# parseablehq/parseable

Hardware: AMD Instinct MI355X
Metric: rows/sec scanned (SELECT...WHERE...GROUP BY, Parseable parquet dialect) (higher is better)
Workload: dtype int64; 1 GPU; c2s; query=SELECT host,count(*),max(latency) WHERE ts BETWEEN ... GROUP BY host, rows_per_gpu=100000000, parallelism=dp1

## Files before the change

parseable_amd/csrc/gpuq.cpp:

```cpp
#include "../../include/gpuq.h"
#include "catalog.h"
#include "where.h"
#include "meta.h"
#include "kernels_api.h"
#include "dev_types.h"
#include "like.h"

#include <hip/hip_runtime.h>
#include <fcntl.h>
#include <sys/mman.h>
#include <sys/stat.h>
#include <unistd.h>

#include <algorithm>
#include <array>
#include <atomic>
#include <functional>
#include <cstring>
#include <thread>
#include <map>
#include <memory>
#include <mutex>
#include <string>
#include <unordered_map>
// ... 175 lines not shown
struct RgRef {
  int file_idx, rg_idx;
  int64_t rows = 0, needed_bytes = 0, total_bytes = 0;
  uint32_t row_start = 0;
};

enum TaskKind { TK_DICT_GID, TK_DICT_VAL, TK_PLAIN_VAL, TK_DELTA_VAL,
                TK_DICT_MASK, TK_BYTES_CONTAINS, TK_POOL_VAL,
                TK_IS_NULL, TK_IS_NOT_NULL,
                TK_N };
constexpr int TK_CTX_SHIFT = 8;
inline int tk_ctx(int kind, int ctx) { return kind | (ctx << TK_CTX_SHIFT); }
inline int tk_kind(int key) { return key & ((1 << TK_CTX_SHIFT) - 1); }
inline int tk_ctx_of(int key) { return key >> TK_CTX_SHIFT; }

struct Partition {
  int device = -1;
  std::vector<RgRef> rgs;
  int64_t n_rows = 0;
  std::vector<ChunkTask> chunks;
  std::vector<DevPage> pages;
  std::map<std::pair<int,int>, std::vector<int32_t>> tasks;
  std::vector<int32_t> remap_pool;
  std::vector<int64_t> dictv_pool;
  std::vector<uint8_t> lut_pool;
  std::vector<std::vector<uint8_t>> lut_pool_x;
  std::vector<DevSeg> segs;
  std::vector<DevBr> brs;
  std::vector<DevPageBr> pagebrs;
  std::vector<DevBrRes> res_lane, res_wave;
  std::vector<DevPiece> piece_pool;
  std::vector<DevSeq> seqs;
  std::vector<DevSeqTile> tiles;
  std::vector<DevLit> lits_wave;
  std::vector<DevCWin> cwins;
  std::vector<uint16_t> cstarts;
  std::map<int, std::pair<uint32_t, uint32_t>> cwin_ranges;
  uint64_t raw_bytes = 0, dec_bytes = 0;
  int64_t bytes_scanned = 0, rowgroup_bytes_total = 0;
  int64_t bytes_cache_hit = 0;
  bool populated = false;
  std::map<int, std::vector<std::pair<int64_t, int64_t>>> pred_ranges;
  std::vector<std::pair<uint64_t, std::vector<uint8_t>>> himgs;

  bool loaded = false;
  hipStream_t stream = nullptr;
  uint8_t *d_raw = nullptr, *d_dec = nullptr;
  DevPage* d_pages = nullptr;
  int32_t* d_remap = nullptr;
  int64_t* d_dictv = nullptr;
  uint8_t* d_lut = nullptr;
  uint8_t* d_mask = nullptr;
  std::vector<uint8_t*> d_fbufs;
  std::vector<uint8_t*> d_wbufs;
  int32_t* d_err = nullptr;
  uint64_t* d_table = nullptr;
  uint64_t* d_fsum = nullptr;
  uint64_t* d_hkeys = nullptr;
  int32_t* d_hgids = nullptr;
  uint32_t* d_hcount = nullptr;
  std::map<int, uint64_t*> d_gid2ref;
// ... 78 lines not shown
  std::vector<Partition> parts;
  int32_t n_groups = 0;
  int32_t n_fsum = 0;
  bool has_hash = false;
  bool needs_cascade = false;
  bool has_numkey = false;
  std::vector<std::string> pinned_keys;
  int64_t m_cache_hit_bytes = 0;
  bool fused_count = false;
  bool fused_valagg = false;
  int valagg_col = -1;
  bool valagg_late = false;
  int valagg_blocks = 1024;
  bool no_fused_valagg = false;
  bool dict_serial = false;
  bool exec_dbg = false;
  std::vector<int> distinct_aggs;
  bool has_tree = false;
  WhereTree where;
  std::vector<int> pred_ctx;
  struct WOr { int node; int ctx; int level; std::vector<int> terms; };
  struct WFold { int node; int ctx; int col; };
  struct WCtx { std::vector<int> ors; };
  std::vector<WCtx> ctxs;
  std::vector<WOr> wors;
  std::vector<WFold> wfolds;
  int n_wbufs = 0;
  int ctx_of(int pidx) const { return has_tree ? pred_ctx[pidx] : 0; }
  bool no_fcount = false;
  struct AggFilter { int agg; int root; int ctx; int depth; };
// ... 22 lines not shown
extern "C" void gpuq_session_destroy(gpuq_ctx* c) { delete c; }
namespace {
thread_local std::string g_null_ctx_error = "null ctx";
}
extern "C" const char* gpuq_last_error(gpuq_ctx* c) {
  return c ? c->last_error.c_str() : g_null_ctx_error.c_str();
}
extern "C" int32_t gpuq_device_count(void) {
  int n = 0;
  if (hipGetDeviceCount(&n) != hipSuccess) return -1;
  return n;
}

namespace {

void read_env_knobs(gpuq_plan* plan) {
  plan->exec_dbg = getenv("GPUQ_PLAN_DEBUG") != nullptr;
  plan->no_fused_valagg = getenv("GPUQ_NO_FUSED_VALAGG") != nullptr;
  plan->no_fcount = getenv("GPUQ_NO_FCOUNT") != nullptr;
  if (const char* e = getenv("GPUQ_VALAGG_BLOCKS"))
    plan->valagg_blocks = std::max(1, atoi(e));
  if (const char* e = getenv("GPUQ_DICT_WALK"))
    plan->dict_serial = strcmp(e, "serial") == 0;
  if (const char* e = getenv("GPUQ_DISTINCT_BITMAP_BITS"))
    plan->distinct_bitmap_bits =
        std::min<uint64_t>(strtoull(e, nullptr, 10), 1ull << 31);
  if (const char* e = getenv("GPUQ_DISTINCT_LDS_BITS"))
    plan->distinct_lds_bits =
        std::min<uint64_t>(strtoull(e, nullptr, 10), 64 * 1024 * 8);
  if (const char* e = getenv("GPUQ_DISTINCT_PAIR_CAP"))
    plan->distinct_pair_cap = (uint32_t)std::min<uint64_t>(
        std::max<uint64_t>(strtoull(e, nullptr, 10), 1), DISTINCT_PAIR_CAP);
  if (const char* e = getenv("GPUQ_DISTINCT_FORCE_HASH"))
    plan->distinct_force_hash = atoi(e) != 0;
}

int find_or_add_col(std::vector<ColPlan>& cols, const std::string& name) {
  for (size_t i = 0; i < cols.size(); i++)
// ... 329 lines not shown
    const std::vector<T>& s = cbs[i].*src;
    for (size_t j = 0; j < s.size(); j++) {
      T e = s[j];
      rebase(e, i);
      dst[off[i] + j] = e;
    }
  });
  return off;
}
template <class C, class T, class B>
std::vector<size_t> merge_stream(std::vector<C>& cbs, std::vector<T> B::*src,
                                 std::vector<T>& dst) {
  return merge_stream(cbs, src, dst, [](T&, size_t) {});
}

Ring::Ring(hipStream_t st) : stream(st) {
  for (int i = 0; i < NBUF; i++) {
    HIP_TRY(hipHostMalloc(&bufs[i], BUFSZ));
    HIP_TRY(hipEventCreate(&evts[i]));
    HIP_TRY(hipEventRecord(evts[i], stream));
  }
}
Ring::~Ring() {
  for (int i = 0; i < NBUF; i++) {
    if (bufs[i]) (void)hipHostFree(bufs[i]);
    if (evts[i]) (void)hipEventDestroy(evts[i]);
  }
}
void Ring::copy_spans(uint8_t* d_dst, const std::vector<Span>& spans) {
  size_t si = 0;
// ... 17 lines not shown
      if (soff == spans[si].len) { si++; soff = 0; }
    }
    parallel_for(fills.size(), [&](size_t f) {
      memcpy(fills[f].dstp, fills[f].src, fills[f].len);
    }, 32);
    HIP_TRY(hipMemcpyAsync(d_dst + dst, bufs[b], filled,
                           hipMemcpyHostToDevice, stream));
    HIP_TRY(hipEventRecord(evts[b], stream));
    dst += filled;
    b = (b + 1) % NBUF;
  }
}
void Ring::copy(void* d_dst, const void* src, size_t len) {
  if (len) copy_spans((uint8_t*)d_dst, {{(const uint8_t*)src, len}});
}

struct DecompRecs {
  std::vector<DevSeg> segs;
  std::vector<DevBr> brs;
  std::vector<DevPageBr> pagebrs;
  std::vector<DevBrRes> res_lane, res_wave;
  std::vector<DevPiece> piece_pool;
  std::vector<DevSeq> seqs;
  std::vector<DevSeqTile> tiles;
  std::vector<DevLit> lits_wave;
  std::vector<std::pair<uint64_t, std::vector<uint8_t>>> himgs;
};

constexpr uint32_t BR_FAR = 16384 / 2;

void plan_decomp_page(DecompRecs& cb, int codec, const uint8_t* praw,
                      uint64_t src_abs, uint64_t dst_abs, uint32_t comp,
                      uint32_t uncomp, bool raw_page,
                      int force = GPUQ_DECOMP_AUTO,
                      gpuq_decomp_stats* st = nullptr) {
  Lz4Plan lp;
  if (st) *st = gpuq_decomp_stats{};
  if (!raw_page && codec == CODEC_SNAPPY) {
    lp = snappy_walk(praw, comp, uncomp);
    if (st) st->n_seq = lp.n_seq;
    if (lp.fallback) {
      std::vector<uint8_t> img(uncomp);
// ... 166 lines not shown
      }
      push_seq(dst_abs + lt.dst, rec, len);
    } else {
      const Lz4Resolved& rr = lp.resolved[ri++];
      if (try_inline(rr, &pat, &period)) {
        push_seq(dst_abs + rr.dst, {src_abs | match_bits(rr.len, period), pat},
                 rr.len);
        if (st) st->n_inl++;
      } else {
        push_resolved(rr);
      }
    }
  }
}

struct DecompDev {
  const uint8_t* d_raw;
  uint8_t* d_dec;
  const DevSeg* d_segs; int n_segs;
  const DevSeq* d_seqs;
  const DevSeqTile* d_tiles; int n_tiles;
  const DevLit* d_lits_wave; int n_lits_wave;
  const DevBrRes* d_res_lane; int64_t n_res_lane;
  const DevBrRes* d_res_wave; int n_res_wave;
  const DevPiece* d_piece_pool;
  const DevBr* d_brs;
  const DevPageBr* d_pagebrs; int n_pagebrs;
  int32_t* d_err;
};

void launch_decompress(hipStream_t st, const DecompDev& d) {
  launch_lz4_seg(st, d.d_raw, d.d_dec, d.d_segs, d.n_segs, d.d_err);
  launch_seq_tile(st, d.d_raw, d.d_dec, d.d_seqs, d.d_tiles, d.n_tiles);
  launch_lit_wave(st, d.d_raw, d.d_dec, d.d_lits_wave, d.n_lits_wave);
  launch_brres_lane(st, d.d_dec, d.d_res_lane, d.d_piece_pool, d.n_res_lane);
  launch_brres_wave(st, d.d_dec, d.d_res_wave, d.d_piece_pool, d.n_res_wave);
  launch_lz4_backrefs(st, d.d_dec, d.d_brs, d.d_pagebrs, d.n_pagebrs);
}

void plan_debug_report(gpuq_plan* plan,
                       std::map<size_t, std::array<int64_t, 3>>& null_dbg,
                       const std::vector<std::array<int64_t, 2>>& leaf_dbg,
                       const std::vector<char>& or_path) {
  fprintf(stderr, "[gpuq plan] fused_count=%d fused_valagg=%d%s\n",
          (int)plan->fused_count, (int)plan->fused_valagg,
          plan->fused_valagg && plan->valagg_late
              ? " (group count checked at execute)" : "");
  for (int ai : plan->distinct_aggs) {
// ... 7 lines not shown
    size_t period_le3 = 0;
    for (const DevSeq& r : pt.seqs) {
      const uint32_t ml = (uint32_t)(r.a >> 49) & 0x1ff;
      const uint32_t n = std::min(ml, (uint32_t)(r.a >> 58));
      for (uint32_t q = 1; q <= 3 && ml; q++) {
        bool ok = true;
        for (uint32_t j = q; j < n && ok; j++)
          ok = (uint8_t)(r.pat >> (j * 8)) == (uint8_t)(r.pat >> ((j - q) * 8));
        if (ok) { period_le3++; break; }
      }
    }
    fprintf(stderr,
            "[gpuq plan] part %zu: rows=%lld chunks=%zu pages=%zu segs=%zu "
            "tiles=%zu tile_recs=%zu period_le3=%zu lits_wave=%zu "
            "res=%zu/%zu pieces=%zu raw=%.2fGB "
            "dec=%.2fGB cwins=%zu\n",
            p, (long long)pt.n_rows, pt.chunks.size(), pt.pages.size(),
            pt.segs.size(), pt.tiles.size(), pt.seqs.size(), period_le3,
            pt.lits_wave.size(), pt.res_lane.size(), pt.res_wave.size(),
            pt.piece_pool.size(), pt.raw_bytes / 1e9, pt.dec_bytes / 1e9,
            pt.cwins.size());
  }
  for (size_t pi = 0; pi < plan->preds.size(); pi++) {
    const auto& pp = plan->preds[pi];
    std::string path;
    if (op_is_like(pp.p.op)) {
      int ci = find_or_add_col(plan->cols, pp.col);
      if (plan->cols[ci].hash_mode) {
        path = "hash";
      } else {
        bool lut = false, win = false;
        int k = plan->ctx_of((int)pi);
        if (k < 0)
          for (auto& f : plan->wfolds)
            if (f.col == ci) k = f.ctx;
        for (auto& part : plan->parts) {
// ... 914 lines not shown
          } else throw std::runtime_error("unsupported encoding for string predicate");
        }
        for (auto& nt : stubs[ti].null_tasks)
          cb.tasks[{tk_ctx(nt.first, nt.second), t.col_idx}].push_back(this_pid);
        cb.pages.push_back(dp);
      }
      if (row_in_rg != (uint32_t)mf.meta.row_groups[t.rg_idx].num_rows)
        throw std::runtime_error("page rows mismatch");
    });

    phase_mark("phase4 lz4 walks");

    {
      const size_t nc = cbs.size();
      merge_stream(cbs, &CB::pages, part.pages);
      merge_stream(cbs, &CB::segs, part.segs);
      const auto o_brs = merge_stream(cbs, &CB::brs, part.brs);
      merge_stream(cbs, &CB::pagebrs, part.pagebrs,
                   [&](DevPageBr& pb, size_t i) {
                     pb.start += (uint32_t)o_brs[i];
                   });
      const auto o_pp = merge_stream(cbs, &CB::piece_pool, part.piece_pool);
      auto piece_rebase = [&](DevBrRes& r, size_t i) {
        r.piece_start += (uint32_t)o_pp[i];
      };
      merge_stream(cbs, &CB::res_lane, part.res_lane, piece_rebase);
      merge_stream(cbs, &CB::res_wave, part.res_wave, piece_rebase);
      const auto o_sq = merge_stream(cbs, &CB::seqs, part.seqs);
      merge_stream(cbs, &CB::tiles, part.tiles,
                   [&](DevSeqTile& t, size_t i) { t.rec0 += o_sq[i]; });
      merge_stream(cbs, &CB::lits_wave, part.lits_wave);
      for (size_t i = 0; i < nc; i++) {
        auto& cb = cbs[i];
        for (auto& [key, ids] : cb.tasks) {
          auto& dstv = part.tasks[key];
          dstv.insert(dstv.end(), ids.begin(), ids.end());
        }
        citems.insert(citems.end(), cb.citems.begin(), cb.citems.end());
        for (auto& h : cb.himgs)
          part.himgs.emplace_back(h.first, std::move(h.second));
      }
    }
    phase_mark("phase5 merge");
    part.dec_bytes += 16384 + 64;

    if (!citems.empty()) {
// ... 276 lines not shown
  if (ctx) ctx->set_error(e.what());
  return nullptr;
}

extern "C" int32_t gpuq_plan_partition_count(gpuq_plan* p) {
  return p ? (int32_t)p->parts.size() : 0;
}

extern "C" int32_t gpuq_plan_load(gpuq_plan* plan, int32_t pi) try {
  if (!plan || pi < 0 || pi >= (int32_t)plan->parts.size()) return -1;
  Partition& part = plan->parts[pi];
  if (part.loaded) return 0;
  int64_t t0 = now_ns();
  HIP_TRY(hipSetDevice(part.device));
  HIP_TRY(hipStreamCreateWithFlags(&part.stream, hipStreamNonBlocking));

  HIP_TRY(hipMalloc(&part.d_raw, std::max<uint64_t>(part.raw_bytes + 8192, 16)));
  HIP_TRY(hipMalloc(&part.d_dec, std::max<uint64_t>(part.dec_bytes, 16)));
  Ring ring(part.stream);
  {
    std::vector<Ring::Span> run;
    uint64_t run_dst = 0, cursor = 0;
    auto flush = [&]() {
      if (!run.empty()) {
        ring.copy_spans(part.d_raw + run_dst, run);
        run.clear();
      }
    };
    for (auto& t : part.chunks) {
      const auto& mf = *plan->files[t.file_idx];
// ... 145 lines not shown
              (void**)&part.d_brs);
  upload_pool(part.pagebrs.data(), part.pagebrs.size() * sizeof(DevPageBr),
              (void**)&part.d_pagebrs);
  upload_pool(part.res_lane.data(), part.res_lane.size() * sizeof(DevBrRes),
              (void**)&part.d_res_lane);
  upload_pool(part.res_wave.data(), part.res_wave.size() * sizeof(DevBrRes),
              (void**)&part.d_res_wave);
  upload_pool(part.piece_pool.data(), part.piece_pool.size() * sizeof(DevPiece),
              (void**)&part.d_piece_pool);
  upload_pool(part.seqs.data(), part.seqs.size() * sizeof(DevSeq),
              (void**)&part.d_seqs);
  upload_pool(part.tiles.data(), part.tiles.size() * sizeof(DevSeqTile),
              (void**)&part.d_tiles);
  upload_pool(part.lits_wave.data(), part.lits_wave.size() * sizeof(DevLit),
              (void**)&part.d_lits_wave);
  upload_pool(part.cwins.data(), part.cwins.size() * sizeof(DevCWin),
              (void**)&part.d_cwins);
  upload_pool(part.cstarts.data(), part.cstarts.size() * sizeof(uint16_t),
              (void**)&part.d_cstarts);
  std::string needle;
  part.needle_off.assign(plan->preds.size(), 0);
  {
    std::string pool;
    for (size_t i = 0; i < plan->preds.size(); i++) {
      if (plan->preds[i].p.lit_kind == GPUQ_LIT_STR) {
        part.needle_off[i] = (uint32_t)pool.size();
        pool += plan->preds[i].str_lit;
        pool.push_back('\0');
      }
    }
// ... 352 lines not shown
      ch->buffers[1] = v;
    }
  }
  s->cursor += k;
  return 0;
} catch (const std::exception& e) {
  auto* s = (ProjState*)st0->private_data;
  s->err = e.what();
  return 1;
}

}

struct ExecEvents {
  hipEvent_t ev0 = nullptr, ev1 = nullptr, decomp = nullptr;
  ExecEvents() = default;
  ExecEvents(const ExecEvents&) = delete;
  ExecEvents& operator=(const ExecEvents&) = delete;
  void create() {
    HIP_TRY(hipEventCreate(&ev0));
    HIP_TRY(hipEventCreate(&ev1));
    HIP_TRY(hipEventCreate(&decomp));
  }
  ~ExecEvents() {
    for (hipEvent_t e : {ev0, ev1, decomp})
      if (e) (void)hipEventDestroy(e);
  }
};

int cmp_mode_of(int op) {
  switch (op) {
    case GPUQ_EQ: return CMP_EQ;
    case GPUQ_NE: return CMP_NE;
    case GPUQ_LT: return CMP_LT;
    case GPUQ_LE: return CMP_LE;
    case GPUQ_GT: return CMP_GT;
    case GPUQ_GE: return CMP_GE;
    default: return -1;
  }
}
// ... 192 lines not shown
  bool cascaded = false;
  std::vector<uint32_t> level_claimed;
  std::vector<char> distinct_bitmap(plan->distinct_aggs.size(), 0);
  auto key_card = [&](int ci) -> int64_t {
    const auto& kc = plan->cols[ci];
    return kc.is_bin ? (int64_t)kc.nbins + 1
           : (kc.hash_mode || kc.numeric_key)
               ? (int64_t)part.hash_claimed[ci] + 1
               : (int64_t)kc.gdict.size() + 1;
  };
  if (plan->fused_count)
    launch_init_table(st, part.d_table, plan->n_groups, (int)plan->aggs.size(),
                      part.d_agg_kind);

  HIP_TRY(hipEventRecord(ev0, st));
  launch_decompress(st, DecompDev{
      part.d_raw, part.d_dec,
      part.d_segs, (int)part.segs.size(),
      part.d_seqs, part.d_tiles, (int)part.tiles.size(),
      part.d_lits_wave, (int)part.lits_wave.size(),
      part.d_res_lane, (int64_t)part.res_lane.size(),
      part.d_res_wave, (int)part.res_wave.size(),
      part.d_piece_pool, part.d_brs,
      part.d_pagebrs, (int)part.pagebrs.size(), part.d_err});
  HIP_TRY(hipEventRecord(ev_decomp, st));

  if (plan->fused_count) {
    int key_col = plan->group_cols[0];
    auto it = part.tasks.find({TK_DICT_GID, key_col});
    if (it != part.tasks.end())
      launch_dict_count(st, part.d_dec, part.d_pages, part.d_ids[it->first],
                        (int)it->second.size(), part.d_remap, part.d_table,
                        plan->n_groups, (int)plan->aggs.size(), part.d_err);
    HIP_TRY(hipEventRecord(ev1, st));
  } else {
  auto run_task = [&](const std::pair<const std::pair<int, int>,
                                      std::vector<int32_t>>& kv,
                      uint8_t* mk) {
    const int kind = tk_kind(kv.first.first), kctx = tk_ctx_of(kv.first.first);
    const int col = kv.first.second;
    int n = (int)kv.second.size();
    int32_t* ids = part.d_ids[kv.first];
    const uint8_t* d_lut = part.d_lut;
    if (plan->exec_dbg &&
        (kind == TK_DICT_GID || kind == TK_DICT_VAL || kind == TK_DICT_MASK))
      fprintf(stderr,
              "[gpuq exec] part %d: dict decode col=%s pages=%d dict_walk=%s\n",
              pi, plan->cols[col].name.c_str(), n,
// ... 87 lines not shown
                          part.d_tmpvalid, mk, nullptr, nullptr,
                          part.d_present, part.d_err);
        break;
      case TK_IS_NULL:
        launch_def_levels(st, part.d_dec, part.d_pages, ids, n,
                          part.d_tmpvalid, nullptr, nullptr, nullptr,
                          part.d_present, part.d_err);
        launch_null_clear_valid(st, part.d_dec, part.d_pages, ids, n,
                                part.d_tmpvalid, mk);
        break;
    }
  };
  for (auto& kv : part.tasks) {
    if (plan->fused_valagg && kv.first.second == plan->valagg_col) continue;
    if (tk_ctx_of(kv.first.first) != 0) continue;
    run_task(kv, part.d_mask);
  }
  if (plan->has_hash || plan->has_numkey) {
    std::vector<int> gid_cols = plan->group_cols;
    for (int ai : plan->distinct_aggs) {
      int ci = plan->aggs[ai].col_idx;
      if (std::find(gid_cols.begin(), gid_cols.end(), ci) == gid_cols.end())
        gid_cols.push_back(ci);
    }
    for (int ci : gid_cols) {
      auto& c = plan->cols[ci];
      if (!c.hash_mode && !c.numeric_key) continue;
      reset_hash_table(part, st, (1ull << HASH_LOG2) + 1);
      auto itv = part.d_valid.find(ci);
      uint8_t* v = itv != part.d_valid.end() ? itv->second : nullptr;
// ... 23 lines not shown
      if (!c.hash_mode || c.lut_preds.empty()) continue;
      for (int pidx : c.lut_preds) {
        if (plan->ctx_of(pidx) != k) continue;
        const auto& pp = plan->preds[pidx];
        int op = cmp_mode_of(pp.p.op);
        if (op < 0) op = cmp_str_like(like_mode(pp.p.op));
        auto itv = part.d_valid.find((int)ci);
        launch_cmp_str(st, part.d_dec, part.d_val[(int)ci],
                       itv != part.d_valid.end() ? itv->second : nullptr,
                       part.d_needle + part.needle_off[pidx],
                       (uint32_t)pp.str_lit.size(), op, mk,
                       part.n_rows);
      }
    }

    for (size_t ci = 0; ci < plan->cols.size(); ci++) {
      auto& c = plan->cols[ci];
      for (int pidx : c.cmp_preds) {
        if (plan->ctx_of(pidx) != k) continue;
        const auto& pp = plan->preds[pidx];
        int mode = pp.p.op == GPUQ_BETWEEN ? CMP_RANGE : cmp_mode_of(pp.p.op);
        if (mode < 0) throw std::runtime_error("bad cmp op");
        int is_f64 = (c.phys == PT_DOUBLE) ? 1 : 0;
        int64_t lo = pp.p.i64[0], hi = pp.p.i64[1];
        if (is_f64) {
          memcpy(&lo, &pp.p.f64[0], 8);
          memcpy(&hi, &pp.p.f64[1], 8);
        }
        auto rit = part.pred_ranges.find(pidx);
        if (rit == part.pred_ranges.end()) continue;
        for (const auto& [row0, nrows] : rit->second)
          launch_cmp_i64(st, part.d_val[(int)ci] + row0,
                         part.d_valid[(int)ci] + row0,
                         lo, hi, mode, pp.p.hi_exclusive, is_f64,
                         mk + row0, nrows);
      }
    }
  };
  row_preds(0, part.d_mask);

  int where_combines = 0;
  std::vector<const uint8_t*> fbuf(plan->filters.size(), nullptr);
  if (plan->has_tree && (need_mask || !plan->filters.empty())) {
    for (size_t b = 1; b < part.d_wbufs.size(); b += 2)
      HIP_TRY(hipMemsetAsync(part.d_wbufs[b], 1, part.n_rows, st));
    std::function<void(int, uint8_t*)> eval_ors;
    auto eval_ctx = [&](int k, uint8_t* mk) {
      for (auto& kv : part.tasks)
        if (tk_ctx_of(kv.first.first) == k) run_task(kv, mk);
      row_preds(k, mk);
      eval_ors(k, mk);
    };
    eval_ors = [&](int k, uint8_t* mk) {
// ... 588 lines not shown
    F(part.d_rowof); F(part.d_rank); F(part.d_scr);
    F(part.d_present); F(part.d_tmpvalid);
    F(part.d_seqs); F(part.d_tiles); F(part.d_lits_wave);
    F(part.d_cwins); F(part.d_cstarts);
    F(part.d_segs); F(part.d_brs); F(part.d_pagebrs);
    F(part.d_res_lane); F(part.d_res_wave); F(part.d_piece_pool);
    F(part.d_keys); F(part.d_keys_sorted); F(part.d_rows);
    F(part.d_rows_sorted); F(part.d_count); F(part.d_sort_temp);
    for (auto& kv : part.d_ids) F(kv.second);
    F(part.d_valagg_ids);
    F(part.d_dbitmap); F(part.d_dcount);
    for (auto* ptr : part.d_dpairs) F(ptr);
    for (auto& kv : part.d_gid) F(kv.second);
    for (auto& kv : part.d_val) F(kv.second);
    for (auto& kv : part.d_valid) F(kv.second);
    if (part.stream) (void)hipStreamDestroy(part.stream);
  }
}

extern "C" void gpuq_plan_destroy(gpuq_plan* p) { delete p; }

namespace {

constexpr uint64_t DEC_PAD = 16384 + 64;
constexpr uint64_t RAW_SLACK = 8192;

void replay_decompress(const uint8_t* raw, uint8_t* dec, const DecompRecs& R) {
  for (const DevSeg& sg : R.segs) {
    const uint8_t* src = raw + sg.src_off;
    uint8_t* dst = dec + sg.dst_off;
// ... 220 lines not shown
  uint8_t* d_dec = B.alloc<uint8_t>(arena);
  int32_t* d_e = B.alloc<int32_t>(4);
  HIP_TRY(hipMemsetAsync(d_dec, sentinel, arena, B.stream));
  HIP_TRY(hipMemsetAsync(d_e, 0, 4, B.stream));
  if (raw_len)
    HIP_TRY(hipMemcpyAsync(d_raw, raw.data(), raw_len, hipMemcpyHostToDevice,
                           B.stream));
  for (const auto& h : R.himgs)
    if (!h.second.empty())
      HIP_TRY(hipMemcpyAsync(d_dec + h.first, h.second.data(), h.second.size(),
                             hipMemcpyHostToDevice, B.stream));
  DecompDev D{
      d_raw, d_dec,
      B.upload(R.segs), (int)R.segs.size(),
      B.upload(R.seqs), B.upload(R.tiles), (int)R.tiles.size(),
      B.upload(R.lits_wave), (int)R.lits_wave.size(),
      B.upload(R.res_lane), (int64_t)R.res_lane.size(),
      B.upload(R.res_wave), (int)R.res_wave.size(),
      B.upload(R.piece_pool), B.upload(R.brs),
      B.upload(R.pagebrs), (int)R.pagebrs.size(), d_e};
  launch_decompress(B.stream, D);
  HIP_TRY(hipGetLastError());
  int32_t err = 0;
  HIP_TRY(hipMemcpyAsync(out, d_dec, arena, hipMemcpyDeviceToHost, B.stream));
  HIP_TRY(hipMemcpyAsync(&err, d_e, 4, hipMemcpyDeviceToHost, B.stream));
  HIP_TRY(hipStreamSynchronize(B.stream));
  if (d_err) *d_err = err;
  return 0;
} catch (const std::exception& e) {
  if (ctx) ctx->set_error(e.what());
// ... 60 lines not shown
```

parseable_amd/csrc/kernels.hip:

```cpp
#include <hip/hip_runtime.h>
#include <cstring>
#include <rocprim/device/device_radix_sort.hpp>
#include "dev_types.h"
#include "like.h"
#include "meta.h"

namespace gpuq {

#define WAVE 64

#define LZ4_RING 16384
#define LZ4_IN 4096

#define SEG_MAX 8192
__global__ void __launch_bounds__(WAVE)
k_lz4_seg(const uint8_t* __restrict__ raw, uint8_t* __restrict__ dec,
          const DevSeg* __restrict__ segs, int n, int32_t* __restrict__ d_error) {
  __shared__ uint8_t seg[SEG_MAX];
  __shared__ uint8_t inbuf[LZ4_IN + 256];
  int si = blockIdx.x;
  if (si >= n) return;
  const DevSeg sg = segs[si];
  const uint8_t* src = raw + sg.src_off;
  uint8_t* dst = dec + sg.dst_off;
// ... 168 lines not shown
  int r = blockIdx.x;
  if (r >= n) return;
  const DevBrRes rec = recs[r];
  uint32_t pat_off = 0;
  for (uint32_t k = 0; k < rec.piece_n; k++) {
    const DevPiece pc = pieces[rec.piece_start + k];
    for (uint32_t base = pat_off; base < rec.len; base += rec.off) {
      uint32_t m = min(pc.len, rec.len - base);
      for (uint32_t j = threadIdx.x; j < m; j += WAVE)
        dec[rec.dst + base + j] = dec[pc.src + j];
    }
    pat_off += pc.len;
  }
}

__global__ void __launch_bounds__(SEQ_TILE_RECS)
k_seq_tile(const uint8_t* __restrict__ raw, uint8_t* __restrict__ dec,
           const DevSeq* __restrict__ seqs,
           const DevSeqTile* __restrict__ tiles, int n) {
  __shared__ __attribute__((aligned(16))) uint8_t stage[SEQ_TILE_BYTES + 16];
  __shared__ uint32_t wtot[SEQ_TILE_RECS / WAVE];
  if (blockIdx.x >= (unsigned)n) return;
  const DevSeqTile T = tiles[blockIdx.x];
  const uint32_t t = threadIdx.x, lane = t & (WAVE - 1);
  const uint32_t out_len = min(T.out_len, SEQ_TILE_BYTES);
  uint8_t* o = dec + T.dst0;
  const uint32_t pad = (uint32_t)((uintptr_t)o & 15);

  DevSeq R{0, 0};
  if (t < T.n_rec) R = seqs[T.rec0 + t];
  const uint32_t lit = (uint32_t)(R.a >> 40) & 0x1ff;
  const uint32_t ml = (uint32_t)(R.a >> 49) & 0x1ff;
  const uint32_t period = (uint32_t)(R.a >> 58);
  const uint32_t len = lit + ml;
  uint32_t incl = len;
#pragma unroll
  for (int d = 1; d < WAVE; d <<= 1) {
    uint32_t y = __shfl_up(incl, d, WAVE);
    if (lane >= (uint32_t)d) incl += y;
  }
  if (lane == WAVE - 1) wtot[t / WAVE] = incl;
  __syncthreads();
  uint32_t off = incl - len;
  for (uint32_t w = 0; w < t / WAVE; w++) off += wtot[w];

  if (off + len <= out_len) {
    uint8_t* sp = stage + pad + off;
    const uint8_t* s = raw + (R.a & ((1ull << 40) - 1));
    for (uint32_t k = 0; k < lit; k += 8) {
      uint64_t w;
      __builtin_memcpy(&w, s + k, 8);
      const uint32_t m = min(8u, lit - k);
      for (uint32_t j = 0; j < m; j++) sp[k + j] = (uint8_t)(w >> (j * 8));
    }
    sp += lit;
    for (uint32_t j = 0, q = 0; j < ml; j++) {
      sp[j] = (uint8_t)(R.pat >> (q * 8));
      if (++q == period) q = 0;
    }
  }
  __syncthreads();

  const uint32_t head = min((16u - pad) & 15u, out_len);
  if (t < head) o[t] = stage[pad + t];
  const uint32_t body = (out_len - head) & ~15u;
  for (uint32_t i = t * 16u; i < body; i += SEQ_TILE_RECS * 16u)
    *(uint4*)(o + head + i) = *(const uint4*)(stage + pad + head + i);
  const uint32_t tl = head + body + t;
  if (tl < out_len) o[tl] = stage[pad + tl];
}
__global__ void __launch_bounds__(WAVE)
k_lit_wave(const uint8_t* __restrict__ raw, uint8_t* __restrict__ dec,
           const DevLit* __restrict__ lits, int n) {
  if (blockIdx.x >= (unsigned)n) return;
  const DevLit L = lits[blockIdx.x];
  const uint8_t* s = raw + (L.a & ((1ull << 40) - 1));
  const uint32_t len = (uint32_t)(L.a >> 40);
  uint8_t* o = dec + L.b;
  uint32_t nw = len / 8;
  for (uint32_t w = threadIdx.x; w < nw; w += WAVE) {
    uint64_t v;
    __builtin_memcpy(&v, s + w * 8, 8);
    __builtin_memcpy(o + w * 8, &v, 8);
  }
// ... 2354 lines not shown
k_mask_or_reset(uint8_t* __restrict__ acc, uint8_t* __restrict__ tmp,
                int64_t n) {
  mask_combine<true>(acc, tmp, n);
}
__global__ void __launch_bounds__(MASKOP_T)
k_mask_and(uint8_t* __restrict__ dst, const uint8_t* __restrict__ acc,
           int64_t n) {
  mask_combine<false>(dst, const_cast<uint8_t*>(acc), n);
}

void launch_lz4_seg(hipStream_t st, const uint8_t* raw, uint8_t* dec,
                    const DevSeg* segs, int n, int32_t* d_err) {
  if (n) hipLaunchKernelGGL(k_lz4_seg, dim3(n), dim3(WAVE), 0, st, raw, dec, segs, n, d_err);
}
void launch_seq_tile(hipStream_t st, const uint8_t* raw, uint8_t* dec,
                     const DevSeq* seqs, const DevSeqTile* tiles, int n) {
  if (n) hipLaunchKernelGGL(k_seq_tile, dim3(n), dim3(SEQ_TILE_RECS), 0, st, raw, dec, seqs, tiles, n);
}
void launch_lit_wave(hipStream_t st, const uint8_t* raw, uint8_t* dec,
                     const DevLit* lits, int n) {
  if (n) hipLaunchKernelGGL(k_lit_wave, dim3(n), dim3(WAVE), 0, st, raw, dec, lits, n);
}
void launch_lz4_backrefs(hipStream_t st, uint8_t* dec, const DevBr* brs,
                         const DevPageBr* pages, int n) {
  if (n) hipLaunchKernelGGL(k_lz4_backrefs, dim3(n), dim3(WAVE), 0, st, dec, brs, pages, n);
}
void launch_brres_lane(hipStream_t st, uint8_t* dec, const DevBrRes* recs,
                       const DevPiece* pieces, int64_t n) {
  if (n) hipLaunchKernelGGL(k_brres_lane, dim3((int)((n + 255) / 256)), dim3(256), 0, st, dec, recs, pieces, n);
}
void launch_brres_wave(hipStream_t st, uint8_t* dec, const DevBrRes* recs,
                       const DevPiece* pieces, int n) {
// ... 390 lines not shown
```

parseable_amd/csrc/kernels_api.h:

```cpp
#pragma once
#include <hip/hip_runtime.h>
#include "dev_types.h"

namespace gpuq {
void launch_lz4_seg(hipStream_t, const uint8_t* raw, uint8_t* dec,
                    const DevSeg*, int n, int32_t* d_err);
void launch_seq_tile(hipStream_t, const uint8_t* raw, uint8_t* dec,
                     const DevSeq* seqs, const DevSeqTile* tiles, int n);
void launch_lit_wave(hipStream_t, const uint8_t* raw, uint8_t* dec,
                     const DevLit* lits, int n);
void launch_lz4_backrefs(hipStream_t, uint8_t* dec, const DevBr*,
                         const DevPageBr*, int n);
void launch_brres_lane(hipStream_t, uint8_t* dec, const DevBrRes*,
                       const DevPiece*, int64_t n);
void launch_brres_wave(hipStream_t, uint8_t* dec, const DevBrRes*,
                       const DevPiece*, int n);
void launch_def_levels(hipStream_t, const uint8_t* dec, const DevPage*,
                       const int32_t* ids, int n, uint8_t* valid,
                       uint8_t* null_mask, uint32_t* rowof, uint32_t* rank,
                       uint32_t* present, int32_t* d_err);
void launch_str_win(hipStream_t, const uint8_t* dec, const DevCWin* wins,
                    int n, const DevPage* pages, const uint16_t* starts_pool,
                    const uint8_t* needle, int nlen, int mode,
                    const uint32_t* rowof, uint8_t* mask);
// ... 101 lines not shown
```

Measured before the change: 33.57 billion rows/s.

## Fork delta-encoded predicate columns onto side stream and batch seq-tile decompression

Filter-only columns whose pages are all delta-bitpacked get their decompression records split into a separate set. On a second stream, that set is decompressed, delta-decoded and compared against the predicate, overlapping with the main-stream decompression of the other columns, and the streams join before any mask step that depends on it. Separately, the seq-tile LZ4 kernel is templated so one block can process K tiles, with K defaulting to 2, which cuts block count and interleaves the prefix scans. This adds a second stream, extra event synchronisation and more shared memory per block, and risks contention between the two streams.

```diff
diff --git a/parseable_amd/csrc/gpuq.cpp b/parseable_amd/csrc/gpuq.cpp
--- a/parseable_amd/csrc/gpuq.cpp
+++ b/parseable_amd/csrc/gpuq.cpp
@@ -213,7 +213,35 @@
 inline int tk_kind(int key) { return key & ((1 << TK_CTX_SHIFT) - 1); }
 inline int tk_ctx_of(int key) { return key >> TK_CTX_SHIFT; }
 
-struct Partition {
+struct DecompRecs {
+  std::vector<DevSeg> segs;
+  std::vector<DevBr> brs;
+  std::vector<DevPageBr> pagebrs;
+  std::vector<DevBrRes> res_lane, res_wave;
+  std::vector<DevPiece> piece_pool;
+  std::vector<DevSeq> seqs;
+  std::vector<DevSeqTile> tiles;
+  std::vector<DevLit> lits_wave;
+  std::vector<std::pair<uint64_t, std::vector<uint8_t>>> himgs;
+};
+
+struct DecompDev {
+  const uint8_t* d_raw;
+  uint8_t* d_dec;
+  const DevSeg* d_segs; int n_segs;
+  const DevSeq* d_seqs;
+  const DevSeqTile* d_tiles; int n_tiles;
+  int seq_batch;
+  const DevLit* d_lits_wave; int n_lits_wave;
+  const DevBrRes* d_res_lane; int64_t n_res_lane;
+  const DevBrRes* d_res_wave; int n_res_wave;
+  const DevPiece* d_piece_pool;
+  const DevBr* d_brs;
+  const DevPageBr* d_pagebrs; int n_pagebrs;
+  int32_t* d_err;
+};
+
+struct Partition : DecompRecs {
   int device = -1;
   std::vector<RgRef> rgs;
   int64_t n_rows = 0;
@@ -224,14 +252,8 @@
   std::vector<int64_t> dictv_pool;
   std::vector<uint8_t> lut_pool;
   std::vector<std::vector<uint8_t>> lut_pool_x;
-  std::vector<DevSeg> segs;
-  std::vector<DevBr> brs;
-  std::vector<DevPageBr> pagebrs;
-  std::vector<DevBrRes> res_lane, res_wave;
-  std::vector<DevPiece> piece_pool;
-  std::vector<DevSeq> seqs;
-  std::vector<DevSeqTile> tiles;
-  std::vector<DevLit> lits_wave;
+  std::vector<int> fork_cols;
+  DecompRecs early;
   std::vector<DevCWin> cwins;
   std::vector<uint16_t> cstarts;
   std::map<int, std::pair<uint32_t, uint32_t>> cwin_ranges;
@@ -240,10 +262,11 @@
   int64_t bytes_cache_hit = 0;
   bool populated = false;
   std::map<int, std::vector<std::pair<int64_t, int64_t>>> pred_ranges;
-  std::vector<std::pair<uint64_t, std::vector<uint8_t>>> himgs;
 
   bool loaded = false;
   hipStream_t stream = nullptr;
+  hipStream_t side = nullptr;
+  DecompDev d_early{};
   uint8_t *d_raw = nullptr, *d_dec = nullptr;
   DevPage* d_pages = nullptr;
   int32_t* d_remap = nullptr;
@@ -352,6 +375,8 @@
   int valagg_blocks = 1024;
   bool no_fused_valagg = false;
   bool dict_serial = false;
+  int seq_tile_batch = SEQ_TILE_BATCH_DEFAULT;
+  bool no_delta_fork = false;
   bool exec_dbg = false;
   std::vector<int> distinct_aggs;
   bool has_tree = false;
@@ -404,6 +429,25 @@
 
 namespace {
 
+int seq_tile_batch_env() {
+  if (const char* e = getenv("GPUQ_SEQ_TILE_BATCH")) {
+    const int k = atoi(e);
+    if (k == 1 || k == 2 || k == 4 || k == 8) return k;
+  }
+  return SEQ_TILE_BATCH_DEFAULT;
+}
+
+bool fork_col(const gpuq_plan& plan, int ci) {
+  const ColPlan& c = plan.cols[ci];
+  if (!c.need_val || c.val_always || c.need_gid || c.hash_mode ||
+      c.numeric_key || c.distinct_val || c.is_bin || c.cmp_preds.empty() ||
+      !c.lut_preds.empty() || !c.null_preds.empty())
+    return false;
+  for (int pidx : c.cmp_preds)
+    if (plan.ctx_of(pidx) != 0 || plan.pred_filter[pidx] >= 0) return false;
+  return true;
+}
+
 void read_env_knobs(gpuq_plan* plan) {
   plan->exec_dbg = getenv("GPUQ_PLAN_DEBUG") != nullptr;
   plan->no_fused_valagg = getenv("GPUQ_NO_FUSED_VALAGG") != nullptr;
@@ -412,6 +456,8 @@
     plan->valagg_blocks = std::max(1, atoi(e));
   if (const char* e = getenv("GPUQ_DICT_WALK"))
     plan->dict_serial = strcmp(e, "serial") == 0;
+  plan->seq_tile_batch = seq_tile_batch_env();
+  plan->no_delta_fork = getenv("GPUQ_NO_DELTA_FORK") != nullptr;
   if (const char* e = getenv("GPUQ_DISTINCT_BITMAP_BITS"))
     plan->distinct_bitmap_bits =
         std::min<uint64_t>(strtoull(e, nullptr, 10), 1ull << 31);
@@ -771,6 +817,24 @@
   return merge_stream(cbs, src, dst, [](T&, size_t) {});
 }
 
+template <class C>
+void merge_decomp_recs(std::vector<C>& cbs, DecompRecs& dst) {
+  merge_stream(cbs, &DecompRecs::segs, dst.segs);
+  const auto o_brs = merge_stream(cbs, &DecompRecs::brs, dst.brs);
+  merge_stream(cbs, &DecompRecs::pagebrs, dst.pagebrs,
+               [&](DevPageBr& pb, size_t i) { pb.start += (uint32_t)o_brs[i]; });
+  const auto o_pp = merge_stream(cbs, &DecompRecs::piece_pool, dst.piece_pool);
+  auto piece_rebase = [&](DevBrRes& r, size_t i) {
+    r.piece_start += (uint32_t)o_pp[i];
+  };
+  merge_stream(cbs, &DecompRecs::res_lane, dst.res_lane, piece_rebase);
+  merge_stream(cbs, &DecompRecs::res_wave, dst.res_wave, piece_rebase);
+  const auto o_sq = merge_stream(cbs, &DecompRecs::seqs, dst.seqs);
+  merge_stream(cbs, &DecompRecs::tiles, dst.tiles,
+               [&](DevSeqTile& t, size_t i) { t.rec0 += o_sq[i]; });
+  merge_stream(cbs, &DecompRecs::lits_wave, dst.lits_wave);
+}
+
 Ring::Ring(hipStream_t st) : stream(st) {
   for (int i = 0; i < NBUF; i++) {
     HIP_TRY(hipHostMalloc(&bufs[i], BUFSZ));
@@ -818,18 +882,6 @@
 void Ring::copy(void* d_dst, const void* src, size_t len) {
   if (len) copy_spans((uint8_t*)d_dst, {{(const uint8_t*)src, len}});
 }
-
-struct DecompRecs {
-  std::vector<DevSeg> segs;
-  std::vector<DevBr> brs;
-  std::vector<DevPageBr> pagebrs;
-  std::vector<DevBrRes> res_lane, res_wave;
-  std::vector<DevPiece> piece_pool;
-  std::vector<DevSeq> seqs;
-  std::vector<DevSeqTile> tiles;
-  std::vector<DevLit> lits_wave;
-  std::vector<std::pair<uint64_t, std::vector<uint8_t>>> himgs;
-};
 
 constexpr uint32_t BR_FAR = 16384 / 2;
 
@@ -1026,24 +1078,10 @@
   }
 }
 
-struct DecompDev {
-  const uint8_t* d_raw;
-  uint8_t* d_dec;
-  const DevSeg* d_segs; int n_segs;
-  const DevSeq* d_seqs;
-  const DevSeqTile* d_tiles; int n_tiles;
-  const DevLit* d_lits_wave; int n_lits_wave;
-  const DevBrRes* d_res_lane; int64_t n_res_lane;
-  const DevBrRes* d_res_wave; int n_res_wave;
-  const DevPiece* d_piece_pool;
-  const DevBr* d_brs;
-  const DevPageBr* d_pagebrs; int n_pagebrs;
-  int32_t* d_err;
-};
-
 void launch_decompress(hipStream_t st, const DecompDev& d) {
   launch_lz4_seg(st, d.d_raw, d.d_dec, d.d_segs, d.n_segs, d.d_err);
-  launch_seq_tile(st, d.d_raw, d.d_dec, d.d_seqs, d.d_tiles, d.n_tiles);
+  launch_seq_tile(st, d.d_raw, d.d_dec, d.d_seqs, d.d_tiles, d.n_tiles,
+                  d.seq_batch);
   launch_lit_wave(st, d.d_raw, d.d_dec, d.d_lits_wave, d.n_lits_wave);
   launch_brres_lane(st, d.d_dec, d.d_res_lane, d.d_piece_pool, d.n_res_lane);
   launch_brres_wave(st, d.d_dec, d.d_res_wave, d.d_piece_pool, d.n_res_wave);
@@ -1081,12 +1119,17 @@
             "[gpuq plan] part %zu: rows=%lld chunks=%zu pages=%zu segs=%zu "
             "tiles=%zu tile_recs=%zu period_le3=%zu lits_wave=%zu "
             "res=%zu/%zu pieces=%zu raw=%.2fGB "
-            "dec=%.2fGB cwins=%zu\n",
+            "dec=%.2fGB cwins=%zu fork_cols=%zu early_segs=%zu "
+            "early_tiles=%zu early_tile_recs=%zu early_lits_wave=%zu "
+            "early_res=%zu/%zu early_pagebrs=%zu\n",
             p, (long long)pt.n_rows, pt.chunks.size(), pt.pages.size(),
             pt.segs.size(), pt.tiles.size(), pt.seqs.size(), period_le3,
             pt.lits_wave.size(), pt.res_lane.size(), pt.res_wave.size(),
             pt.piece_pool.size(), pt.raw_bytes / 1e9, pt.dec_bytes / 1e9,
-            pt.cwins.size());
+            pt.cwins.size(), pt.fork_cols.size(), pt.early.segs.size(),
+            pt.early.tiles.size(), pt.early.seqs.size(),
+            pt.early.lits_wave.size(), pt.early.res_lane.size(),
+            pt.early.res_wave.size(), pt.early.pagebrs.size());
   }
   for (size_t pi = 0; pi < plan->preds.size(); pi++) {
     const auto& pp = plan->preds[pi];
@@ -2031,22 +2074,33 @@
     {
       const size_t nc = cbs.size();
       merge_stream(cbs, &CB::pages, part.pages);
-      merge_stream(cbs, &CB::segs, part.segs);
-      const auto o_brs = merge_stream(cbs, &CB::brs, part.brs);
-      merge_stream(cbs, &CB::pagebrs, part.pagebrs,
-                   [&](DevPageBr& pb, size_t i) {
-                     pb.start += (uint32_t)o_brs[i];
-                   });
-      const auto o_pp = merge_stream(cbs, &CB::piece_pool, part.piece_pool);
-      auto piece_rebase = [&](DevBrRes& r, size_t i) {
-        r.piece_start += (uint32_t)o_pp[i];
-      };
-      merge_stream(cbs, &CB::res_lane, part.res_lane, piece_rebase);
-      merge_stream(cbs, &CB::res_wave, part.res_wave, piece_rebase);
-      const auto o_sq = merge_stream(cbs, &CB::seqs, part.seqs);
-      merge_stream(cbs, &CB::tiles, part.tiles,
-                   [&](DevSeqTile& t, size_t i) { t.rec0 += o_sq[i]; });
-      merge_stream(cbs, &CB::lits_wave, part.lits_wave);
+      std::vector<DecompRecs> ecbs(nc);
+      if (!plan->no_delta_fork) {
+        std::vector<char> forks(plan->cols.size(), 0), seen = forks;
+        for (size_t ci = 0; ci < plan->cols.size(); ci++)
+          forks[ci] = fork_col(*plan, (int)ci);
+        for (size_t i = 0; i < nc; i++) {
+          const auto& t = part.chunks[i];
+          if (!forks[t.col_idx] || !stubs[i].need_val_decode) continue;
+          seen[t.col_idx] = 1;
+          for (const auto& pi : t.pages)
+            if (pi.type == PAGE_DATA && pi.encoding != ENC_DELTA_BP)
+              forks[t.col_idx] = 0;
+        }
+        for (size_t ci = 0; ci < plan->cols.size(); ci++)
+          if (forks[ci] && seen[ci]) part.fork_cols.push_back((int)ci);
+        for (size_t i = 0; i < nc; i++) {
+          const int ci = part.chunks[i].col_idx;
+          if (!forks[ci] || !seen[ci] || !stubs[i].need_val_decode) continue;
+          DecompRecs& all = cbs[i];
+          auto himgs = std::move(all.himgs);
+          ecbs[i] = std::move(all);
+          all = DecompRecs{};
+          all.himgs = std::move(himgs);
+        }
+      }
+      merge_decomp_recs(cbs, part);
+      merge_decomp_recs(ecbs, part.early);
       for (size_t i = 0; i < nc; i++) {
         auto& cb = cbs[i];
         for (auto& [key, ids] : cb.tasks) {
@@ -2353,6 +2407,8 @@
   int64_t t0 = now_ns();
   HIP_TRY(hipSetDevice(part.device));
   HIP_TRY(hipStreamCreateWithFlags(&part.stream, hipStreamNonBlocking));
+  if (!part.fork_cols.empty())
+    HIP_TRY(hipStreamCreateWithFlags(&part.side, hipStreamNonBlocking));
 
   HIP_TRY(hipMalloc(&part.d_raw, std::max<uint64_t>(part.raw_bytes + 8192, 16)));
   HIP_TRY(hipMalloc(&part.d_dec, std::max<uint64_t>(part.dec_bytes, 16)));
@@ -2528,6 +2584,23 @@
               (void**)&part.d_tiles);
   upload_pool(part.lits_wave.data(), part.lits_wave.size() * sizeof(DevLit),
               (void**)&part.d_lits_wave);
+  if (!part.fork_cols.empty()) {
+    const DecompRecs& E = part.early;
+    DecompDev& D = part.d_early;
+    auto up = [&](const auto& v, auto** dst) {
+      upload_pool(v.data(), v.size() * sizeof(v[0]), (void**)dst);
+    };
+    up(E.segs, &D.d_segs); D.n_segs = (int)E.segs.size();
+    up(E.seqs, &D.d_seqs);
+    up(E.tiles, &D.d_tiles); D.n_tiles = (int)E.tiles.size();
+    up(E.lits_wave, &D.d_lits_wave); D.n_lits_wave = (int)E.lits_wave.size();
+    up(E.res_lane, &D.d_res_lane); D.n_res_lane = (int64_t)E.res_lane.size();
+    up(E.res_wave, &D.d_res_wave); D.n_res_wave = (int)E.res_wave.size();
+    up(E.piece_pool, &D.d_piece_pool);
+    up(E.brs, &D.d_brs);
+    up(E.pagebrs, &D.d_pagebrs); D.n_pagebrs = (int)E.pagebrs.size();
+    D.seq_batch = plan->seq_tile_batch;
+  }
   upload_pool(part.cwins.data(), part.cwins.size() * sizeof(DevCWin),
               (void**)&part.d_cwins);
   upload_pool(part.cstarts.data(), part.cstarts.size() * sizeof(uint16_t),
@@ -2910,6 +2983,8 @@
 
 struct ExecEvents {
   hipEvent_t ev0 = nullptr, ev1 = nullptr, decomp = nullptr;
+  hipEvent_t fork = nullptr, join = nullptr;
+  hipStream_t side = nullptr;
   ExecEvents() = default;
   ExecEvents(const ExecEvents&) = delete;
   ExecEvents& operator=(const ExecEvents&) = delete;
@@ -2918,8 +2993,22 @@
     HIP_TRY(hipEventCreate(&ev1));
     HIP_TRY(hipEventCreate(&decomp));
   }
+  void fork_side(hipStream_t main, hipStream_t sd) {
+    HIP_TRY(hipEventCreateWithFlags(&fork, hipEventDisableTiming));
+    HIP_TRY(hipEventCreateWithFlags(&join, hipEventDisableTiming));
+    HIP_TRY(hipEventRecord(fork, main));
+    HIP_TRY(hipStreamWaitEvent(sd, fork, 0));
+    side = sd;
+  }
+  void join_side(hipStream_t main) {
+    if (!side) return;
+    HIP_TRY(hipEventRecord(join, side));
+    HIP_TRY(hipStreamWaitEvent(main, join, 0));
+    side = nullptr;
+  }
   ~ExecEvents() {
-    for (hipEvent_t e : {ev0, ev1, decomp})
+    if (side) (void)hipStreamSynchronize(side);
+    for (hipEvent_t e : {ev0, ev1, decomp, fork, join})
       if (e) (void)hipEventDestroy(e);
   }
 };
@@ -3142,10 +3231,56 @@
                       part.d_agg_kind);
 
   HIP_TRY(hipEventRecord(ev0, st));
+  auto cmp_col = [&](hipStream_t s, int ci, int k, uint8_t* mk) {
+    auto& c = plan->cols[ci];
+    for (int pidx : c.cmp_preds) {
+      if (plan->ctx_of(pidx) != k) continue;
+      const auto& pp = plan->preds[pidx];
+      int mode = pp.p.op == GPUQ_BETWEEN ? CMP_RANGE : cmp_mode_of(pp.p.op);
+      if (mode < 0) throw std::runtime_error("bad cmp op");
+      int is_f64 = (c.phys == PT_DOUBLE) ? 1 : 0;
+      int64_t lo = pp.p.i64[0], hi = pp.p.i64[1];
+      if (is_f64) {
+        memcpy(&lo, &pp.p.f64[0], 8);
+        memcpy(&hi, &pp.p.f64[1], 8);
+      }
+      auto rit = part.pred_ranges.find(pidx);
+      if (rit == part.pred_ranges.end()) continue;
+      for (const auto& [row0, nrows] : rit->second)
+        launch_cmp_i64(s, part.d_val[ci] + row0, part.d_valid[ci] + row0,
+                       lo, hi, mode, pp.p.hi_exclusive, is_f64,
+                       mk + row0, nrows);
+    }
+  };
+  const bool forked = !part.fork_cols.empty();
+  auto is_fork_col = [&](int ci) {
+    return std::find(part.fork_cols.begin(), part.fork_cols.end(), ci) !=
+           part.fork_cols.end();
+  };
+  if (forked) {
+    hipStream_t sd = part.side;
+    events.fork_side(st, sd);
+    DecompDev E = part.d_early;
+    E.d_raw = part.d_raw;
+    E.d_dec = part.d_dec;
+    E.d_err = part.d_err;
+    launch_decompress(sd, E);
+    for (int ci : part.fork_cols) {
+      auto it = part.tasks.find({TK_DELTA_VAL, ci});
+      if (it != part.tasks.end())
+        launch_delta_i64(sd, part.d_dec, part.d_pages, part.d_ids[it->first],
+                         (int)it->second.size(), part.d_val[ci],
+                         part.d_valid[ci], part.d_err);
+      cmp_col(sd, ci, 0, part.d_mask);
+    }
+    if (plan->exec_dbg)
+      fprintf(stderr, "[gpuq exec] part %d: delta fork cols=%zu\n", (int)pi,
+              part.fork_cols.size());
+  }
   launch_decompress(st, DecompDev{
       part.d_raw, part.d_dec,
       part.d_segs, (int)part.segs.size(),
-      part.d_seqs, part.d_tiles, (int)part.tiles.size(),
+      part.d_seqs, part.d_tiles, (int)part.tiles.size(), plan->seq_tile_batch,
       part.d_lits_wave, (int)part.lits_wave.size(),
       part.d_res_lane, (int64_t)part.res_lane.size(),
       part.d_res_wave, (int)part.res_wave.size(),
@@ -3160,6 +3295,7 @@
       launch_dict_count(st, part.d_dec, part.d_pages, part.d_ids[it->first],
                         (int)it->second.size(), part.d_remap, part.d_table,
                         plan->n_groups, (int)plan->aggs.size(), part.d_err);
+    events.join_side(st);
     HIP_TRY(hipEventRecord(ev1, st));
   } else {
   auto run_task = [&](const std::pair<const std::pair<int, int>,
@@ -3277,6 +3413,12 @@
   for (auto& kv : part.tasks) {
     if (plan->fused_valagg && kv.first.second == plan->valagg_col) continue;
     if (tk_ctx_of(kv.first.first) != 0) continue;
+    const int kind = tk_kind(kv.first.first);
+    if (forked && kind == TK_DELTA_VAL && is_fork_col(kv.first.second))
+      continue;
+    if (kind == TK_DICT_MASK || kind == TK_BYTES_CONTAINS ||
+        kind == TK_IS_NULL || kind == TK_IS_NOT_NULL)
+      events.join_side(st);
     run_task(kv, part.d_mask);
   }
   if (plan->has_hash || plan->has_numkey) {
@@ -3330,29 +3472,10 @@
       }
     }
 
-    for (size_t ci = 0; ci < plan->cols.size(); ci++) {
-      auto& c = plan->cols[ci];
-      for (int pidx : c.cmp_preds) {
-        if (plan->ctx_of(pidx) != k) continue;
-        const auto& pp = plan->preds[pidx];
-        int mode = pp.p.op == GPUQ_BETWEEN ? CMP_RANGE : cmp_mode_of(pp.p.op);
-        if (mode < 0) throw std::runtime_error("bad cmp op");
-        int is_f64 = (c.phys == PT_DOUBLE) ? 1 : 0;
-        int64_t lo = pp.p.i64[0], hi = pp.p.i64[1];
-        if (is_f64) {
-          memcpy(&lo, &pp.p.f64[0], 8);
-          memcpy(&hi, &pp.p.f64[1], 8);
-        }
-        auto rit = part.pred_ranges.find(pidx);
-        if (rit == part.pred_ranges.end()) continue;
-        for (const auto& [row0, nrows] : rit->second)
-          launch_cmp_i64(st, part.d_val[(int)ci] + row0,
-                         part.d_valid[(int)ci] + row0,
-                         lo, hi, mode, pp.p.hi_exclusive, is_f64,
-                         mk + row0, nrows);
-      }
-    }
+    for (size_t ci = 0; ci < plan->cols.size(); ci++)
+      if (!forked || !is_fork_col((int)ci)) cmp_col(st, (int)ci, k, mk);
   };
+  events.join_side(st);
   row_preds(0, part.d_mask);
 
   int where_combines = 0;
@@ -3971,6 +4094,14 @@
     for (auto& kv : part.d_gid) F(kv.second);
     for (auto& kv : part.d_val) F(kv.second);
     for (auto& kv : part.d_valid) F(kv.second);
+    const DecompDev& E = part.d_early;
+    for (const void* ptr : {(const void*)E.d_segs, (const void*)E.d_seqs,
+                            (const void*)E.d_tiles, (const void*)E.d_lits_wave,
+                            (const void*)E.d_res_lane, (const void*)E.d_res_wave,
+                            (const void*)E.d_piece_pool, (const void*)E.d_brs,
+                            (const void*)E.d_pagebrs})
+      F(const_cast<void*>(ptr));
+    if (part.side) (void)hipStreamDestroy(part.side);
     if (part.stream) (void)hipStreamDestroy(part.stream);
   }
 }
@@ -4221,6 +4352,7 @@
       d_raw, d_dec,
       B.upload(R.segs), (int)R.segs.size(),
       B.upload(R.seqs), B.upload(R.tiles), (int)R.tiles.size(),
+      seq_tile_batch_env(),
       B.upload(R.lits_wave), (int)R.lits_wave.size(),
       B.upload(R.res_lane), (int64_t)R.res_lane.size(),
       B.upload(R.res_wave), (int)R.res_wave.size(),
diff --git a/parseable_amd/csrc/kernels.hip b/parseable_amd/csrc/kernels.hip
--- a/parseable_amd/csrc/kernels.hip
+++ b/parseable_amd/csrc/kernels.hip
@@ -1,5 +1,6 @@
 #include <hip/hip_runtime.h>
 #include <cstring>
+#include <stdexcept>
 #include <rocprim/device/device_radix_sort.hpp>
 #include "dev_types.h"
 #include "like.h"
@@ -206,14 +207,41 @@
   }
 }
 
-__global__ void __launch_bounds__(SEQ_TILE_RECS)
-k_seq_tile(const uint8_t* __restrict__ raw, uint8_t* __restrict__ dec,
-           const DevSeq* __restrict__ seqs,
-           const DevSeqTile* __restrict__ tiles, int n) {
-  __shared__ __attribute__((aligned(16))) uint8_t stage[SEQ_TILE_BYTES + 16];
-  __shared__ uint32_t wtot[SEQ_TILE_RECS / WAVE];
-  if (blockIdx.x >= (unsigned)n) return;
-  const DevSeqTile T = tiles[blockIdx.x];
+
+__device__ __forceinline__ void seq_flush(uint8_t* __restrict__ o,
+                                          const uint8_t* st, uint32_t out_len,
+                                          uint32_t t) {
+  const uint32_t pad = (uint32_t)((uintptr_t)o & 15);
+  const uint32_t head = min((16u - pad) & 15u, out_len);
+  if (t < head) o[t] = st[t];
+  const uint32_t body = (out_len - head) & ~15u;
+  for (uint32_t i = t * 16u; i < body; i += SEQ_TILE_RECS * 16u)
+    *(uint4*)(o + head + i) = *(const uint4*)(st + head + i);
+  const uint32_t tl = head + body + t;
+  if (tl < out_len) o[tl] = st[tl];
+}
+
+__device__ __forceinline__ void seq_put(uint8_t* sp, const uint8_t* s,
+                                        uint64_t w0, uint32_t lit, uint32_t ml,
+                                        uint32_t period, uint64_t pat) {
+  uint64_t w = w0;
+  for (uint32_t k = 0; k < lit; k += 8) {
+    if (k) __builtin_memcpy(&w, s + k, 8);
+    const uint32_t m = min(8u, lit - k);
+    for (uint32_t j = 0; j < m; j++) sp[k + j] = (uint8_t)(w >> (j * 8));
+  }
+  sp += lit;
+  for (uint32_t j = 0, q = 0; j < ml; j++) {
+    sp[j] = (uint8_t)(pat >> (q * 8));
+    if (++q == period) q = 0;
+  }
+}
+
+__device__ __forceinline__ void seq_tile_one(const uint8_t* __restrict__ raw,
+                                             uint8_t* __restrict__ dec,
+                                             const DevSeq* __restrict__ seqs,
+                                             const DevSeqTile& T,
+                                             uint8_t* stage, uint32_t* wtot) {
   const uint32_t t = threadIdx.x, lane = t & (WAVE - 1);
   const uint32_t out_len = min(T.out_len, SEQ_TILE_BYTES);
   uint8_t* o = dec + T.dst0;
@@ -225,6 +253,9 @@
   const uint32_t ml = (uint32_t)(R.a >> 49) & 0x1ff;
   const uint32_t period = (uint32_t)(R.a >> 58);
   const uint32_t len = lit + ml;
+  const uint8_t* s = raw + (R.a & ((1ull << 40) - 1));
+  uint64_t w0;
+  __builtin_memcpy(&w0, s, 8);
   uint32_t incl = len;
 #pragma unroll
   for (int d = 1; d < WAVE; d <<= 1) {
@@ -236,30 +267,87 @@
   uint32_t off = incl - len;
   for (uint32_t w = 0; w < t / WAVE; w++) off += wtot[w];
 
-  if (off + len <= out_len) {
-    uint8_t* sp = stage + pad + off;
-    const uint8_t* s = raw + (R.a & ((1ull << 40) - 1));
-    for (uint32_t k = 0; k < lit; k += 8) {
-      uint64_t w;
-      __builtin_memcpy(&w, s + k, 8);
-      const uint32_t m = min(8u, lit - k);
-      for (uint32_t j = 0; j < m; j++) sp[k + j] = (uint8_t)(w >> (j * 8));
-    }
-    sp += lit;
-    for (uint32_t j = 0, q = 0; j < ml; j++) {
-      sp[j] = (uint8_t)(R.pat >> (q * 8));
-      if (++q == period) q = 0;
-    }
-  }
+  if (off + len <= out_len)
+    seq_put(stage + pad + off, s, w0, lit, ml, period, R.pat);
   __syncthreads();
-
-  const uint32_t head = min((16u - pad) & 15u, out_len);
-  if (t < head) o[t] = stage[pad + t];
-  const uint32_t body = (out_len - head) & ~15u;
-  for (uint32_t i = t * 16u; i < body; i += SEQ_TILE_RECS * 16u)
-    *(uint4*)(o + head + i) = *(const uint4*)(stage + pad + head + i);
-  const uint32_t tl = head + body + t;
-  if (tl < out_len) o[tl] = stage[pad + tl];
+  seq_flush(o, stage + pad, out_len, t);
+}
+
+template <int K>
+__global__ void __launch_bounds__(SEQ_TILE_RECS)
+k_seq_tile(const uint8_t* __restrict__ raw, uint8_t* __restrict__ dec,
+           const DevSeq* __restrict__ seqs,
+           const DevSeqTile* __restrict__ tiles, int n) {
+  constexpr uint32_t NW = SEQ_TILE_RECS / WAVE;
+  constexpr uint32_t STAGE = SEQ_TILE_BYTES + 16 * K;
+  __shared__ __attribute__((aligned(16))) uint8_t stage[STAGE];
+  __shared__ uint32_t wtot[K][NW];
+  const int64_t b0 = (int64_t)blockIdx.x * K;
+  if (b0 >= n) return;
+  if constexpr (K == 1) {
+    seq_tile_one(raw, dec, seqs, tiles[b0], stage, wtot[0]);
+    return;
+  } else {
+  const uint32_t t = threadIdx.x, lane = t & (WAVE - 1);
+
+  DevSeqTile T[K];
+  uint32_t sbase[K];
+  uint32_t top = 0;
+#pragma unroll
+  for (int k = 0; k < K; k++) {
+    T[k] = b0 + k < n ? tiles[b0 + k] : DevSeqTile{0, 0, 0, 0};
+    T[k].out_len = min(T[k].out_len, SEQ_TILE_BYTES);
+    sbase[k] = top + (uint32_t)((uintptr_t)(dec + T[k].dst0) & 15);
+    top = (sbase[k] + T[k].out_len + 15u) & ~15u;
+  }
+  if (top > STAGE) {
+    for (int k = 0; k < K; k++)
+      if (b0 + k < n) seq_tile_one(raw, dec, seqs, T[k], stage, wtot[0]);
+    return;
+  }
+
+  DevSeq R[K];
+#pragma unroll
+  for (int k = 0; k < K; k++) {
+    R[k] = DevSeq{0, 0};
+    if (t < T[k].n_rec) R[k] = seqs[T[k].rec0 + t];
+  }
+  uint32_t lit[K], ml[K], incl[K];
+  uint64_t w0[K];
+#pragma unroll
+  for (int k = 0; k < K; k++) {
+    lit[k] = (uint32_t)(R[k].a >> 40) & 0x1ff;
+    ml[k] = (uint32_t)(R[k].a >> 49) & 0x1ff;
+    incl[k] = lit[k] + ml[k];
+    __builtin_memcpy(&w0[k], raw + (R[k].a & ((1ull << 40) - 1)), 8);
+  }
+#pragma unroll
+  for (int d = 1; d < WAVE; d <<= 1) {
+#pragma unroll
+    for (int k = 0; k < K; k++) {
+      uint32_t y = __shfl_up(incl[k], d, WAVE);
+      if (lane >= (uint32_t)d) incl[k] += y;
+    }
+  }
+  if (lane == WAVE - 1) {
+#pragma unroll
+    for (int k = 0; k < K; k++) wtot[k][t / WAVE] = incl[k];
+  }
+  __syncthreads();
+#pragma unroll
+  for (int k = 0; k < K; k++) {
+    const uint32_t len = lit[k] + ml[k];
+    uint32_t off = incl[k] - len;
+    for (uint32_t w = 0; w < t / WAVE; w++) off += wtot[k][w];
+    if (off + len <= T[k].out_len)
+      seq_put(stage + sbase[k] + off, raw + (R[k].a & ((1ull << 40) - 1)),
+              w0[k], lit[k], ml[k], (uint32_t)(R[k].a >> 58), R[k].pat);
+  }
+  __syncthreads();
+#pragma unroll
+  for (int k = 0; k < K; k++)
+    seq_flush(dec + T[k].dst0, stage + sbase[k], T[k].out_len, t);
+  }
 }
 __global__ void __launch_bounds__(WAVE)
 k_lit_wave(const uint8_t* __restrict__ raw, uint8_t* __restrict__ dec,
@@ -2644,8 +2732,20 @@
   if (n) hipLaunchKernelGGL(k_lz4_seg, dim3(n), dim3(WAVE), 0, st, raw, dec, segs, n, d_err);
 }
 void launch_seq_tile(hipStream_t st, const uint8_t* raw, uint8_t* dec,
-                     const DevSeq* seqs, const DevSeqTile* tiles, int n) {
-  if (n) hipLaunchKernelGGL(k_seq_tile, dim3(n), dim3(SEQ_TILE_RECS), 0, st, raw, dec, seqs, tiles, n);
+                     const DevSeq* seqs, const DevSeqTile* tiles, int n,
+                     int batch) {
+  if (!n) return;
+  auto go = [&](auto kern, int k) {
+    hipLaunchKernelGGL(kern, dim3((n + k - 1) / k), dim3(SEQ_TILE_RECS), 0, st,
+                       raw, dec, seqs, tiles, n);
+  };
+  switch (batch) {
+    case 1: go(k_seq_tile<1>, 1); break;
+    case 2: go(k_seq_tile<2>, 2); break;
+    case 4: go(k_seq_tile<4>, 4); break;
+    case 8: go(k_seq_tile<8>, 8); break;
+    default: throw std::runtime_error("launch_seq_tile: bad batch");
+  }
 }
 void launch_lit_wave(hipStream_t st, const uint8_t* raw, uint8_t* dec,
                      const DevLit* lits, int n) {
diff --git a/parseable_amd/csrc/kernels_api.h b/parseable_amd/csrc/kernels_api.h
--- a/parseable_amd/csrc/kernels_api.h
+++ b/parseable_amd/csrc/kernels_api.h
@@ -5,8 +5,10 @@
 namespace gpuq {
 void launch_lz4_seg(hipStream_t, const uint8_t* raw, uint8_t* dec,
                     const DevSeg*, int n, int32_t* d_err);
+constexpr int SEQ_TILE_BATCH_DEFAULT = 2;
 void launch_seq_tile(hipStream_t, const uint8_t* raw, uint8_t* dec,
-                     const DevSeq* seqs, const DevSeqTile* tiles, int n);
+                     const DevSeq* seqs, const DevSeqTile* tiles, int n,
+                     int batch);
 void launch_lit_wave(hipStream_t, const uint8_t* raw, uint8_t* dec,
                      const DevLit* lits, int n);
 void launch_lz4_backrefs(hipStream_t, uint8_t* dec, const DevBr*,
```

Result: faster. 36.54 billion rows/s (median of 6 runs) (+8.9%).
